# DecaYale/RNNPose

Measured on AMD Instinct MI355X. Metric: pose-refine iters/sec (640x480, B=8, 3x8 recurrent), higher is better.
Workload: dtype f32 (convolutions and volume build: fp16x3-split MFMA, fp32-class accuracy; LM: f64)

## Files before the change

### include/rnnpose_hip.h

```cpp
#ifndef RNNPOSE_HIP_H
#define RNNPOSE_HIP_H

#include <stddef.h>
#include <stdint.h>

#ifdef __cplusplus
extern "C" {
#endif

typedef void* rnnpose_stream_t;

#define RNNPOSE_ABI_VERSION 4
#define RNNPOSE_MAX_LEVELS 4

int rnnpose_abi_version(void);
const char* rnnpose_last_error(void);
int rnnpose_device_info(int dev, char* h_name, int name_len, int* h_cus);

int rnnpose_corr_pyramid_layout(int B, int h, int w, int levels, int64_t* h_offsets ,
                                int* h_hl , int* h_wl );
int rnnpose_corr_pyramid_f32(const float* fmap1, const float* fmap2, int B, int C, int h, int w,
                             int levels, float* pyramid, rnnpose_stream_t stream);
size_t rnnpose_corr_pyramid_f16x3_workspace_bytes(int B, int C, int h, int w);
int rnnpose_corr_pyramid_f16x3(const float* fmap1, const float* fmap2, int layout, int B, int C, int h, int w, int levels,
// ... 191 lines not shown
                             long long ldo, rnnpose_stream_t stream);
long long rnnpose_point_norm_workspace_bytes(int n, int c);
int rnnpose_point_norm_stats_f32(const float* x, int n, int c, long long ldx, float eps, void* workspace, long long workspace_bytes,
                                 float* mean_rstd, rnnpose_stream_t stream);
int rnnpose_point_norm_apply_f32(const float* x, int n, int c, long long ldx, const float* mean_rstd, const float* res, long long ldr,
                                 const float* res_mean_rstd, int leaky, float slope, float* out, long long ldo,
                                 rnnpose_stream_t stream);
int rnnpose_point_maxpool_f32(const float* x, int n_s, int c, long long ldx, const int* idx, int n_q, int width, float* out,
                              long long ldo, rnnpose_stream_t stream);
int rnnpose_point_gather_rows_f32(const float* x, int n_s, int c, long long ldx, const int* idx, int n_q, int idx_ld, float* out,
                                  long long ldo, rnnpose_stream_t stream);
int rnnpose_point_l2_normalize_f32(const float* x, int n, int c, long long ldx, float* out, long long ldo, rnnpose_stream_t stream);
int rnnpose_grid_voxel_keys_f32(const float* points, int n, float ox, float oy, float oz, float dl, long long nx, long long ny,
                                long long* keys, rnnpose_stream_t stream);
int rnnpose_radius_count_f32(const float* queries, int n_q, const float* supports, const int* q_start, const int* s_start,
                             int n_clouds, float radius, int* counts, rnnpose_stream_t stream);
int rnnpose_radius_neighbors_f32(const float* queries, int n_q, const float* supports, const int* q_start, const int* s_start,
                                 int n_clouds, float radius, const long long* offsets, int* cand_idx, float* cand_d2, int width,
                                 int* out, rnnpose_stream_t stream);
size_t rnnpose_conv1x1_resident_packed_bytes(int c_in);
int rnnpose_conv1x1_resident_pack_f16x3(const float* weight, int c_out, int c_in, float w_scale, void* packed,
                                        rnnpose_stream_t stream);
int rnnpose_conv1x1_resident_f16x3(const float* x, int x_c_stride, int x_c_offset, int c_in, const void* w_packed,
                                   const float* bias, float a_scale, float w_scale, int relu, long long n_pixels, float* dst,
                                   int dst_c_stride, int dst_c_offset, int dst_split, rnnpose_stream_t stream);
int rnnpose_corr_lookup_convc1_f16x3(const float* pyramid, const float* coords, int B, int b0, int b1, int h, int w, int levels,
                                     int radius, const void* w_packed, const float* bias, float a_scale, float w_scale, int relu,
                                     float* dst, int dst_c_stride, int dst_c_offset, int dst_split, rnnpose_stream_t stream);
size_t rnnpose_mask_upsample_packed_bytes(void);
int rnnpose_mask_upsample_pack_f16x3(const float* weight, float post_scale, float w_scale, void* packed, rnnpose_stream_t stream);
int rnnpose_mask_upsample_f16x3(const float* x, int x_c_stride, int x_c_offset, const void* w_packed, int c_out,
                                const float* bias, float a_scale, float w_scale, const float* flow_lr, int B, int h, int w,
                                float* flow_up, rnnpose_stream_t stream);

size_t rnnpose_instnorm_workspace_bytes(int B, int HW, int C);
int rnnpose_instnorm_nhwc_f32(const float* x, int B, int HW, int C, float eps, int relu, const float* residual,
                              void* workspace, size_t workspace_bytes, float* mean_rstd, float* out,
                              rnnpose_stream_t stream);
int rnnpose_instnorm_tiles_nhwc_f32(const float* x, int B, int HW, int C, float eps, int relu, const float* residual,
                                    const float* residual_mean_rstd, int residual_relu, const double* tile_stats,
                                    int tiles_per_image, float* mean_rstd, float* out,
                                    rnnpose_stream_t stream);

int rnnpose_nn_search_f32(const float* ref_pts, const float* que_pts, int* idxs, int b, int pn1, int pn2, int dim,
                          int exclude_self, rnnpose_stream_t stream);
void findNearestPointIdxLauncher(float* ref_pts, float* que_pts, int* idxs, int b, int pn1, int pn2, int dim,
                                 int exclude_self);

size_t rnnpose_pose_metrics_workspace_bytes(int B, int P);
int rnnpose_pose_metrics_f64(const float* model, int P, const float* pose_pred, const float* pose_gt, const float* K, int B,
                             int symmetric, void* workspace, size_t workspace_bytes, double* out, rnnpose_stream_t stream);

size_t rnnpose_bop_sym_dist_workspace_bytes(int B, int S);
int rnnpose_bop_sym_dist_f64(const float* model, int P, const float* sym, int S, const float* pose_est, const float* pose_gt,
                             const float* K, int B, void* workspace, size_t workspace_bytes, double* out, rnnpose_stream_t stream);
size_t rnnpose_bop_vsd_workspace_bytes(int B, int H, int W, int NT);
int rnnpose_bop_vsd_f64(const float* depth_est, const float* depth_gt, const float* depth_obs, int S_obs, const int* src_index,
                        const float* K, const float* diameter, int B, int H, int W, double delta, const double* taus, int NT,
                        void* workspace, size_t workspace_bytes, long long* counts, double* err, rnnpose_stream_t stream);

size_t rnnpose_pointcloud_depth_workspace_bytes(int B, int H, int W);
int rnnpose_pointcloud_depth_f32(const float* verts, const int* vert_offsets, int max_verts, const float* T, const float* K, int B,
                                 int H, int W, void* workspace, size_t workspace_bytes, float* out, rnnpose_stream_t stream);
int rnnpose_mask_bbox_f32(const float* depth, int B, int H, int W, int* bbox, rnnpose_stream_t stream);
int rnnpose_zoom_crop_params_f32(const int* bbox, const float* K, const float* T, int B, int H, int W, int crop_h, int crop_w,
                                 float margin_ratio, float* theta, float* K_crop, rnnpose_stream_t stream);
// ... 33 lines not shown
```

### rnnpose_amd/_lib.py

```python
from __future__ import annotations

import ctypes as C
import os

_PKG = os.path.dirname(os.path.abspath(__file__))
ABI_VERSION = 4
LIB_PATH = os.environ.get("RNNPOSE_LIB") or os.path.join(_PKG, "lib", "librnnpose_hip.so")

_p = C.c_void_p
_i = C.c_int
_f = C.c_float
_d = C.c_double
_z = C.c_size_t
_ll = C.c_longlong

class ConvSrc(C.Structure):
    _fields_ = [("ptr", C.c_void_p), ("c_stride", C.c_int), ("c_offset", C.c_int), ("c_count", C.c_int)]


class ConvDesc(C.Structure):
    _fields_ = [("src", ConvSrc * 4), ("n_src", C.c_int), ("B", C.c_int), ("H", C.c_int), ("W", C.c_int),
                ("kh", C.c_int), ("kw", C.c_int), ("stride", C.c_int), ("w_packed", C.c_void_p), ("bias", C.c_void_p),
                ("c_out", C.c_int), ("a_scale", C.c_float), ("w_scale", C.c_float), ("epilogue", C.c_int),
                ("dst", C.c_void_p), ("dst_c_stride", C.c_int), ("dst_c_offset", C.c_int),
# ... 67 lines not shown
    "rnnpose_corr_lookup_nhwc_part_f32": (_i, [_p, _p, _i, _i, _i, _i, _i, _i, _i, _p, _p]),
    "rnnpose_nchw_to_nhwc_f32": (_i, [_p, _i, _i, _i, _p, _i, _i, _p]),
    "rnnpose_nhwc_to_nchw_f32": (_i, [_p, _i, _i, _i, _i, _i, _p, _p]),
    "rnnpose_flow_prep_f32": (_i, [_p, _i, _i, _i, _i, _p, _p, _i, _i, _p]),
    "rnnpose_flow_conv7x7_relu_f32": (_i, [_p, _p, _p, _i, _i, _i, _i, _p, _i, _i, _p]),
    "rnnpose_flow_features_f32": (_i, [_p, _i, _p, _p, _i, _i, _i, _i, _p, _i, _i, _p, _i, _i, _i, _i, _f, _p]),
    "rnnpose_flow_features_induced_f32": (_i, [_p, _p, _p, _i, _i, _f, _p, _p, _i, _i, _i, _i, _p, _i, _i, _p, _i, _i, _i, _i, _f, _p]),
    "rnnpose_corr_lookup_induced_nhwc_part_f32": (_i, [_p, _p, _p, _p, _i, _i, _f, _i, _i, _i, _i, _i, _i, _i, _p, _p, _p]),
    "rnnpose_split_hl_f32": (_i, [_p, _i, _i, _ll, _i, _f, _p, _i, _i, _p]),
    "rnnpose_maxpool2x2_nhwc_f32": (_i, [_p, _i, _i, _i, _i, _i, _i, _p, _i, _i, _p]),
    "rnnpose_upsample2x_bilinear_nhwc_f32": (_i, [_p, _i, _i, _i, _i, _i, _i, _p, _i, _p, _i, _i, _p]),
    "rnnpose_pixel_head_nhwc_f32": (_i, [_p, _i, _i, _i, _i, _i, _p, _i, _p, _p, _i, _i, _p, _p]),
    "rnnpose_point_row_sum_f32": (_i, [_p, _i, _i, _ll, _p, _p]),
    "rnnpose_kpconv_aggregate_f32": (_i, [_p, _i, _p, _i, _p, _i, _p, _i, _f, _p, _i, _ll, _p, _p, _p]),
    "rnnpose_point_linear_f32": (_i, [_p, _i, _i, _ll, _p, _i, _p, _p, _ll, _p]),
    "rnnpose_point_norm_workspace_bytes": (_ll, [_i, _i]),
    "rnnpose_point_norm_stats_f32": (_i, [_p, _i, _i, _ll, _f, _p, _ll, _p, _p]),
    "rnnpose_point_norm_apply_f32": (_i, [_p, _i, _i, _ll, _p, _p, _ll, _p, _i, _f, _p, _ll, _p]),
    "rnnpose_point_maxpool_f32": (_i, [_p, _i, _i, _ll, _p, _i, _i, _p, _ll, _p]),
    "rnnpose_point_gather_rows_f32": (_i, [_p, _i, _i, _ll, _p, _i, _i, _p, _ll, _p]),
    "rnnpose_point_l2_normalize_f32": (_i, [_p, _i, _i, _ll, _p, _ll, _p]),
    "rnnpose_grid_voxel_keys_f32": (_i, [_p, _i, _f, _f, _f, _f, _ll, _ll, _p, _p]),
    "rnnpose_radius_count_f32": (_i, [_p, _i, _p, _p, _p, _i, _f, _p, _p]),
    "rnnpose_radius_neighbors_f32": (_i, [_p, _i, _p, _p, _p, _i, _f, _p, _p, _p, _i, _p, _p]),
    "rnnpose_flow_head_out_f32": (_i, [_p, _i, _i, _i, _p, _p, _p, _i, _i, _i, _p, _p, _p, _p]),
    "rnnpose_convex_upsample_nhwc_f32": (_i, [_p, _p, _i, _i, _i, _p, _p]),
    "rnnpose_mask_upsample_f16x3": (_i, [_p, _i, _i, _p, _i, _p, _f, _f, _p, _i, _i, _i, _p, _p]),
    "rnnpose_mask_upsample_packed_bytes": (_z, []),
    "rnnpose_conv1x1_resident_packed_bytes": (_z, [_i]),
    "rnnpose_conv1x1_resident_pack_f16x3": (_i, [_p, _i, _i, _f, _p, _p]),
    "rnnpose_conv1x1_resident_f16x3": (_i, [_p, _i, _i, _i, _p, _p, _f, _f, _i, _ll, _p, _i, _i, _i, _p]),
    "rnnpose_corr_lookup_convc1_f16x3": (_i, [_p, _p, _i, _i, _i, _i, _i, _i, _i, _p, _p, _f, _f, _i, _p, _i, _i, _i, _p]),
    "rnnpose_mask_upsample_pack_f16x3": (_i, [_p, _f, _f, _p, _p]),
    "rnnpose_instnorm_workspace_bytes": (_z, [_i, _i, _i]),
    "rnnpose_instnorm_tiles_nhwc_f32": (_i, [_p, _i, _i, _i, _f, _i, _p, _p, _i, _p, _i, _p, _p, _p]),
    "rnnpose_instnorm_nhwc_f32": (_i, [_p, _i, _i, _i, _f, _i, _p, _p, _z, _p, _p, _p]),
    "rnnpose_nn_search_f32": (_i, [_p, _p, _p, _i, _i, _i, _i, _i, _p]),
    "findNearestPointIdxLauncher": (None, [_p, _p, _p, _i, _i, _i, _i, _i]),
    "rnnpose_pointcloud_depth_workspace_bytes": (_z, [_i, _i, _i]),
    "rnnpose_pointcloud_depth_f32": (_i, [_p, _p, _i, _p, _p, _i, _i, _i, _p, _z, _p, _p]),
    "rnnpose_mask_bbox_f32": (_i, [_p, _i, _i, _i, _p, _p]),
    "rnnpose_zoom_crop_params_f32": (_i, [_p, _p, _p, _i, _i, _i, _i, _i, _f, _p, _p, _p]),
    "rnnpose_zoom_crop_f32": (_i, [_p, _p, _i, _i, _i, _i, _i, _i, _p, _p, _p]),
    "rnnpose_zoom_crop_indexed_f32": (_i, [_p, _p, _p, _i, _i, _i, _i, _i, _i, _i, _p, _p, _p]),
    "rnnpose_raster_workspace_bytes": (_z, [_i, _i, _i]),
    "rnnpose_raster_mesh_f32": (_i, [_p, _p, _p, _p, _p, _i, _p, _p, _i, _i, _i, _f, _f, _i, _p, _z, _p]),
    "rnnpose_raster_resolve_f32": (_i, [_p, _p, _p, _p, _p, _p, _i, _i, _i, _f, _f, _i, _p, _p, _p, _i, _p, _i, _i, _f, _p, _p, _p, _p]),
    "rnnpose_raster_resolve_tex_f32": (_i, [_p, _p, _p, _p, _p, _p, _i, _i, _i, _f, _f, _i, _p, _p, _p, _i, _p, _p, _p, _p, _p, _p, _p, _p,
                                            _i, _f, _p, _p, _p, _p]),
    "rnnpose_raster_occlusion_f32": (_i, [_p, _p, _p, _p, _p, _i, _p, _p, _i, _i, _i, _f, _f, _p, _p, _i, _f, _p, _p, _z, _p, _p, _p, _p]),
    "rnnpose_pose_metrics_workspace_bytes": (_z, [_i, _i]),
    "rnnpose_pose_metrics_f64": (_i, [_p, _i, _p, _p, _p, _i, _i, _p, _z, _p, _p]),
    "rnnpose_bop_sym_dist_workspace_bytes": (_z, [_i, _i]),
    "rnnpose_bop_sym_dist_f64": (_i, [_p, _i, _p, _i, _p, _p, _p, _i, _p, _z, _p, _p]),
    "rnnpose_bop_vsd_workspace_bytes": (_z, [_i, _i, _i, _i]),
    "rnnpose_bop_vsd_f64": (_i, [_p, _p, _p, _i, _p, _p, _p, _i, _i, _i, _d, _p, _i, _p, _z, _p, _p, _p]),
}

_lib = None


def load() -> C.CDLL:
    global _lib
    if _lib is not None:
        return _lib
    if not os.path.exists(LIB_PATH):
# ... 30 lines not shown
```

### rnnpose_amd/build.py

```python
from __future__ import annotations

import glob
import hashlib
import os
import subprocess
import sys

PKG = os.path.dirname(os.path.abspath(__file__))
ROOT = os.path.dirname(PKG)
CSRC = os.path.join(PKG, "csrc")
LIBDIR = os.path.join(PKG, "lib")
LIB = os.path.join(LIBDIR, "librnnpose_hip.so")
STAMP = os.path.join(LIBDIR, "librnnpose_hip.stamp")
ARCH = "gfx950"
FLAGS = ["-O3", "-std=c++17", "-fPIC", "-shared", f"--offload-arch={ARCH}", "-fno-gpu-rdc", "-Wall",
         "-Wno-unused-function", "-Wno-unused-variable", "-DNDEBUG", "-fno-slp-vectorize"]
PER_FILE_FLAGS = {}
FLAGS += os.environ.get("RNNPOSE_HIPCC_EXTRA", "").split()


def sources():
    return sorted(glob.glob(os.path.join(CSRC, "*.hip")))


TRAFFIC_KERNEL_FILES = ("conv_igemm.hip", "conv_strip.hip", "conv_strip_r32.hip", "conv_strip_r96.hip", "conv_strip_p1.hip", "corr_pyramid.hip")


def source_digest() -> str:
    h = hashlib.sha256()
    files = [os.path.join(CSRC, f) for f in TRAFFIC_KERNEL_FILES] + sorted(glob.glob(os.path.join(CSRC, "*.hpp"))) + \
        sorted(glob.glob(os.path.join(CSRC, "*.cuh")))
    for f in files:
        h.update(os.path.relpath(f, ROOT).encode())
        with open(f, "rb") as fh:
            h.update(fh.read())
    h.update(" ".join(FLAGS).encode())
    h.update(repr(sorted((k, v) for k, v in PER_FILE_FLAGS.items() if k in TRAFFIC_KERNEL_FILES)).encode())
    return h.hexdigest()


def _digest() -> str:
    h = hashlib.sha256()
    files = sources() + sorted(glob.glob(os.path.join(CSRC, "*.hpp"))) + sorted(glob.glob(os.path.join(CSRC, "*.cuh")))
    files.append(os.path.join(ROOT, "include", "rnnpose_hip.h"))
    for f in files:
        h.update(os.path.relpath(f, ROOT).encode())
        with open(f, "rb") as fh:
            h.update(fh.read())
    h.update(" ".join(FLAGS).encode())
    h.update(repr(sorted(PER_FILE_FLAGS.items())).encode())
    return h.hexdigest()


def hipcc() -> str:
    for c in (os.environ.get("HIPCC"), "/opt/rocm/bin/hipcc", "hipcc"):
        if c and (os.path.isabs(c) and os.path.exists(c) or not os.path.isabs(c)):
            return c
    raise RuntimeError("hipcc not found")


def build(force: bool = False, verbose: bool = False) -> str:
    import fcntl
    os.makedirs(LIBDIR, exist_ok=True)
    dig = _digest()
    if not force and os.path.exists(LIB) and os.path.exists(STAMP) and open(STAMP).read().strip() == dig:
        return LIB
    with open(os.path.join(LIBDIR, ".build.lock"), "w") as lock:
        fcntl.flock(lock, fcntl.LOCK_EX)
        try:
            if not force and os.path.exists(LIB) and os.path.exists(STAMP) and open(STAMP).read().strip() == dig:
                return LIB
            return _build_locked(dig, verbose)
        finally:
            fcntl.flock(lock, fcntl.LOCK_UN)


# ... 41 lines not shown
```

### rnnpose_amd/csrc/nhwc_ops.hip

```cpp
#define RP_CONTRACT_LOCAL 1
#include "common.hpp"
#include "f16x3.cuh"
#include "induced.cuh"

namespace {

__global__ __launch_bounds__(256) void nchw_to_nhwc_kernel(const float* __restrict__ src, float* __restrict__ dst, int C,
                                                           int HW, int dst_cs, int dst_co) {
  __shared__ float tile[32][33];
  const int b = blockIdx.z;
  const int p0 = blockIdx.x * 32, c0 = blockIdx.y * 32;
  const int tx = threadIdx.x & 31, ty = threadIdx.x >> 5;
#pragma unroll
  for (int r = 0; r < 4; ++r) {
    const int c = c0 + ty + 8 * r, pp = p0 + tx;
    tile[ty + 8 * r][tx] = (c < C && pp < HW) ? src[(static_cast<long long>(b) * C + c) * HW + pp] : 0.f;
  }
  __syncthreads();
#pragma unroll
  for (int r = 0; r < 4; ++r) {
    const int pp = p0 + ty + 8 * r, c = c0 + tx;
    if (c < C && pp < HW) dst[(static_cast<long long>(b) * HW + pp) * dst_cs + dst_co + c] = tile[tx][ty + 8 * r];
  }
}
// ... 1342 lines not shown

int rnnpose_grid_voxel_keys_f32(const float* points, int n, float ox, float oy, float oz, float dl, long long nx, long long ny,
                                long long* keys, rnnpose_stream_t stream) {
  const char* fn = "rnnpose_grid_voxel_keys_f32";
  RP_REQUIRE(points && keys, fn, "null pointer");
  RP_REQUIRE(n > 0 && dl > 0.f && nx > 0 && ny > 0, fn, "bad size (n, nx, ny > 0, dl > 0)");
  hipLaunchKernelGGL(grid_keys_kernel, dim3(rp::cdiv(n, 256)), dim3(256), 0, rp::as_stream(stream), points, n, ox, oy, oz, dl, nx, ny,
                     reinterpret_cast<i64*>(keys));
  return rp::check_launch(fn);
}

int rnnpose_radius_count_f32(const float* queries, int n_q, const float* supports, const int* q_start, const int* s_start,
                             int n_clouds, float radius, int* counts, rnnpose_stream_t stream) {
  const char* fn = "rnnpose_radius_count_f32";
  RP_REQUIRE(queries && supports && q_start && s_start && counts, fn, "null pointer");
  RP_REQUIRE(n_q > 0 && n_clouds > 0, fn, "bad size (n_q, n_clouds > 0)");
  hipLaunchKernelGGL(radius_kernel<0>, dim3(rp::cdiv(n_q, 256)), dim3(256), 0, rp::as_stream(stream), queries, n_q, supports, q_start,
                     s_start, n_clouds, radius, counts, nullptr, nullptr, nullptr, 0, nullptr);
  return rp::check_launch(fn);
}

int rnnpose_radius_neighbors_f32(const float* queries, int n_q, const float* supports, const int* q_start, const int* s_start,
                                 int n_clouds, float radius, const long long* offsets, int* cand_idx, float* cand_d2, int width,
                                 int* out, rnnpose_stream_t stream) {
  const char* fn = "rnnpose_radius_neighbors_f32";
  RP_REQUIRE(queries && supports && q_start && s_start && offsets && cand_idx && cand_d2 && out, fn, "null pointer");
  RP_REQUIRE(n_q > 0 && n_clouds > 0 && width > 0, fn, "bad size (n_q, n_clouds, width > 0)");
  hipLaunchKernelGGL(radius_kernel<1>, dim3(rp::cdiv(n_q, 256)), dim3(256), 0, rp::as_stream(stream), queries, n_q, supports, q_start,
                     s_start, n_clouds, radius, nullptr, reinterpret_cast<const i64*>(offsets), cand_idx, cand_d2, width, out);
  return rp::check_launch(fn);
}

}
```

### rnnpose_amd/engine.py

```python
from __future__ import annotations

import torch

from . import env, ops, streams


class UpdateEngine:
    def __init__(self, update_block):
        self.blk = update_block
        self._key = None
        self._w = None
        self._buf_key = None
        self._b = None
        self._sets = {}
        self.epoch = 0
        self._ksws = {}
        self.split_batch = env.flag("RNNPOSE_SPLIT_BATCH", True)
        self.side_stream = env.flag("RNNPOSE_SIDE_STREAM", False)
        self.parts = env.number("RNNPOSE_PARTS", 2)
        self.parts_forced = env.text("RNNPOSE_PARTS") is not None
        self.fused_mask = env.flag("RNNPOSE_FUSED_MASK", True)
        self.resident_1x1 = env.flag("RNNPOSE_RESIDENT_1X1", True)
        self.fused_lookup = env.flag("RNNPOSE_FUSED_LOOKUP", False)
        self.fused_induced = env.flag("RNNPOSE_FUSED_INDUCED", False)
        self.ksplit = env.flag("RNNPOSE_KSPLIT", True)
        self.hl = env.flag("RNNPOSE_SPLIT_TENSORS", True)
        self.single_product = False
        self.tile = {k: int(v) for k, v in (kv.split("=") for kv in filter(None, env.text("RNNPOSE_CONV_TILE", "").split(",")))}

    def _params(self):
        b = self.blk
        e, g = b.encoder, b.gru
        return [e.convc1, e.convc2, e.convf1, e.convf2, e.conv, g.convz1, g.convr1, g.convq1, g.convz2, g.convr2,
                g.convq2, b.flow_head.conv1, b.flow_head.conv2, b.mask[0], b.mask[2]]

    def param_key(self):
        return ops.param_key(self._params())

    def refresh(self):
        self._weights()
        return self._key

    def _weights(self):
        key = self.param_key()
        if key == self._key:
            return self._w
        b = self.blk
        e, g = b.encoder, b.gru
        cat = lambda *t: torch.cat([x.detach() for x in t], 0)
        hm = lambda wt: torch.cat([wt[:, :128], wt[:, 256:]], 1).contiguous()
        zero = lambda n: torch.zeros(n, device=g.convz1.weight.device, dtype=torch.float32)
        P = ops.PackedConv
        w = dict(
            convc1=P(e.convc1.weight, e.convc1.bias, [e.convc1.weight.shape[1]]),
            convc1r=ops.PackedConv1x1(e.convc1.weight, e.convc1.bias) if ops.PackedConv1x1.fits(e.convc1.weight) else None,
            convc2=P(e.convc2.weight, e.convc2.bias, [256]),
            convf1_wt=e.convf1.weight.detach().float().reshape(e.convf1.weight.shape[0], 98).t().contiguous(),
            convf1_b=e.convf1.bias.detach().float().contiguous(),
            convf2=P(e.convf2.weight, e.convf2.bias, [128]),
            conv=P(e.conv.weight, e.conv.bias, [256]),
            zr=P(hm(cat(g.convz1.weight, g.convr1.weight)), cat(g.convz1.bias, g.convr1.bias), [128, 128]),
            q=P(hm(g.convq1.weight), g.convq1.bias, [128, 128]),
            zr2=P(hm(cat(g.convz2.weight, g.convr2.weight)), cat(g.convz2.bias, g.convr2.bias), [128, 128]),
            q2=P(hm(g.convq2.weight), g.convq2.bias, [128, 128]),
            inp1=P(cat(g.convz1.weight, g.convr1.weight, g.convq1.weight)[:, 128:256].contiguous(), zero(384), [128]),
            inp2=P(cat(g.convz2.weight, g.convr2.weight, g.convq2.weight)[:, 128:256].contiguous(), zero(384), [128]),
            heads=P(cat(b.flow_head.conv1.weight, b.mask[0].weight), cat(b.flow_head.conv1.bias, b.mask[0].bias), [128]),
            mask2=P(b.mask[2].weight, b.mask[2].bias, [256], post_scale=0.25),
            mask2u=ops.PackedMaskHead(b.mask[2].weight, b.mask[2].bias, post_scale=0.25),
            flow2_w=b.flow_head.conv2.weight.detach().float().contiguous(),
            flow2_b=b.flow_head.conv2.bias.detach().float().contiguous(),
        )
        self._key, self._w = key, w
        return w

    MAX_SETS = 4

    def _buffers(self, B, h, w, device):
        key = (B, h, w, str(device))
        if key != self._buf_key:
            st = self._sets.pop(key, None)
            if st is None:
                z = lambda c: torch.zeros(B, h, w, c, device=device, dtype=torch.float32)
                st = dict(corr=z(324), cor1=z(256), corflo=z(256), flow4=z(4), flo1=z(128), motion=z(128), hA=z(128),
                          hB=z(128), inp=z(128), inp1=z(384), inp2=z(384), z=z(128), rh=z(128), heads=z(512), delta=z(2), flow_lr=z(2),
                          mask=z(576), coords1=torch.zeros(B, 2, h, w, device=device))
                if self.hl:
                    st.update(hA_s=z(128), hB_s=z(128), inp_s=z(128))
                if len(self._sets) >= self.MAX_SETS:
                    self._sets.pop(next(iter(self._sets)))
                    self.epoch += 1
            self._sets[key] = st
# ... 85 lines not shown

    def step(self, corr_fn, coords1, tail=None, flow_up=None):
        B, _, h, w = coords1.shape
        main = torch.cuda.current_stream()
        if flow_up is None:
            flow_up = torch.empty(B, 2, 8 * h, 8 * w, device=coords1.device, dtype=torch.float32)
        hv = self.halves(B)

        def half(b0, b1, st):
            yield from self.half_gen(corr_fn, coords1[b0:b1], B, b0, b1, st, flow_up[b0:b1], single=len(hv) == 1)
            if tail is not None:
                tail(b0, b1, flow_up[b0:b1])

        jobs = []
        for i, (b0, b1) in enumerate(hv):
            st = main if i == 0 else streams.helper_stream(coords1.device, i)
            jobs.append((half(b0, b1, st), st))
        streams.run_interleaved(jobs, main)
        return self._b["coords1"], flow_up

    def _chain_gen(self, W, b, coords1, main, side, flow_is_delta=False, want_mask=False, have_cor1=False, induced=None):
        mask_here = want_mask or not self.fused_mask
        hl = self.hl
        tl = self.tile.get
        R = ops.EPI_RELU

        ks_main = b.get("_ksws")
        ks_side = b.get("_ksws_side") if side is not None else ks_main

        def c(name, srcs, dst, epi, hl_out=False, ks=None, **kw):
            ops.conv2d_nhwc(W[name], srcs, dst, epi, src_hl=hl, dst_hl=hl and hl_out, tile=tl(name, 0),
                            ksplit_ws=ks_main if ks is None else ks, single_product=self.single_product, **kw)
        def flow_chain():
            if induced is not None:
                ops.flow_features_induced(induced, W["convf1_wt"], W["convf1_b"], b["flo1"], b["motion"], 126, out_split=hl, motion_split=hl,
                                          a_scale=ops.A_SCALE)
            else:
                ops.flow_features(coords1, W["convf1_wt"], W["convf1_b"], b["flo1"], b["motion"], 126, subtract_grid=not flow_is_delta,
                                  out_split=hl, motion_split=hl, a_scale=ops.A_SCALE)
            yield
            c("convf2", [(b["flo1"], 0)], (b["corflo"], 192), R, hl_out=True, ks=ks_side)
            yield

        join = None
        if side is None:
            yield from flow_chain()
        else:
            join = streams.side_branch(main, side, lambda: streams.drain(flow_chain()))
        if have_cor1:
            pass
        elif self.resident_1x1 and W["convc1r"] is not None:
            ops.conv1x1_resident(W["convc1r"], (b["corr"], 0), (b["cor1"], 0), relu=True, dst_split=hl)
            yield
        else:
            ops.conv2d_nhwc(W["convc1"], [(b["corr"], 0)], (b["cor1"], 0), R, dst_hl=hl, single_product=self.single_product)
            yield
        c("convc2", [(b["cor1"], 0)], (b["corflo"], 0), R, hl_out=True)
        yield
        if join is not None:
            main.wait_event(join)
        c("conv", [(b["corflo"], 0)], (b["motion"], 0), R, hl_out=True)
        yield
        hs = (lambda k: b[k + "_s"]) if hl else (lambda k: b[k])
        hx = lambda hbuf: [(hbuf, 0), (b["motion"], 0)]
        sp = (lambda k: dict(dst_split=(b[k + "_s"], 0))) if hl else (lambda k: {})
        c("zr", hx(hs("hA")), (b["z"], 0), ops.EPI_GRU_ZR, aux0=(b["hA"], 0), dst2=(b["rh"], 0), dst2_hl=hl, gru_c=128, add_map=(b["inp1"], 0))
# ... 165 lines not shown
```

### rnnpose_amd/ops.py

```python
from __future__ import annotations

import ctypes as C
from contextlib import contextmanager

import torch

from . import _lib, env

F32 = torch.float32
F64 = torch.float64

_prof = None


_event_pool = []


@contextmanager
def profile(names=None):
    global _prof
    prev = _prof
    rec = {"_only": set(names) if names else None, "_next": 0}
    _prof = rec
    try:
# ... 814 lines not shown
    _launch("rnnpose_nchw_to_nhwc_f32", _ptr(src), B, Cc, H * W, _ptr(dst), dst.shape[3], c_offset, _stream())
    return dst


def nhwc_to_nchw(src, c_offset: int = 0, c_count: int | None = None, out=None):
    B, H, W, Cs = src.shape
    c_count = Cs - c_offset if c_count is None else c_count
    dst = out if out is not None else torch.empty(B, c_count, H, W, device=src.device, dtype=F32)
    _launch("rnnpose_nhwc_to_nchw_f32", _ptr(src), B, c_count, H * W, Cs, c_offset, _ptr(dst), _stream())
    return dst


def flow_prep(coords1, flow4, motion, motion_c_offset, subtract_grid: bool = True):
    B, _, h, w = coords1.shape
    _launch("rnnpose_flow_prep_f32", _ptr(coords1), int(subtract_grid), B, h, w, _ptr(flow4), _ptr(motion), motion.shape[3],
            motion_c_offset, _stream())


def flow_conv7x7_relu(flow4, w_t, bias, out, out_c_offset=0):
    B, h, w, _ = flow4.shape
    c_out = w_t.shape[1]
    _launch("rnnpose_flow_conv7x7_relu_f32", _ptr(flow4), _ptr(w_t), _ptr(bias), B, h, w, c_out, _ptr(out), out.shape[-1],
            out_c_offset, _stream(), work=2.0 * 98 * c_out * B * h * w)
    return out


def flow_features(coords1, w_t, bias, out, motion, motion_c_offset, out_c_offset=0, subtract_grid: bool = True,
                  out_split: bool = False, motion_split: bool = False, a_scale: float = 8.0):
    B, _, h, w = coords1.shape
    c_out = w_t.shape[1]
    _launch("rnnpose_flow_features_f32", _ptr(coords1), int(subtract_grid), _ptr(w_t), _ptr(bias), B, h, w, c_out, _ptr(out),
            out.shape[-1], out_c_offset, _ptr(motion), motion.shape[3], motion_c_offset, int(bool(out_split)), int(bool(motion_split)),
            float(a_scale), _stream(), work=2.0 * 98 * c_out * B * h * w)
    return out


def split_hl(src, dst=None, src_c_offset: int = 0, c_count: int | None = None, dst_c_offset: int = 0, a_scale: float = 8.0):
    _nhwc(src, "src")
    B, H, W, Cs = src.shape
    c_count = Cs - src_c_offset if c_count is None else c_count
    if dst is None:
        dst = torch.empty(B, H, W, c_count, device=src.device, dtype=F32)
    _lib.call("rnnpose_split_hl_f32", _ptr(src), Cs, int(src_c_offset), B * H * W, int(c_count), float(a_scale), _ptr(dst),
              dst.shape[3], int(dst_c_offset), _stream())
    return dst


def unsplit_hl(t, a_scale: float = 8.0):
    sh = t.shape
    v = t.contiguous().view(torch.float16).view(*sh[:-1], sh[-1] // 8, 2, 8).float()
    return ((v[..., 0, :] + v[..., 1, :]) / a_scale).reshape(sh)


def flow_head_out(x, x_c_offset, c_in, weight, bias, coords1, delta, coords1_out, flow_lr):
    B, h, w, cs = x.shape
    _launch("rnnpose_flow_head_out_f32", _ptr(x), cs, x_c_offset, c_in, _ptr(weight), _ptr(bias), _ptr(coords1), B, h, w,
            _ptr(delta), _ptr(coords1_out), _ptr(flow_lr), _stream())


def convex_upsample_nhwc(flow_lr, mask, out=None):
    B, h, w, _ = mask.shape
    if out is None:
        out = torch.empty(B, 2, 8 * h, 8 * w, device=mask.device, dtype=F32)
    _launch("rnnpose_convex_upsample_nhwc_f32", _ptr(flow_lr), _ptr(mask), B, h, w, _ptr(out), _stream(),
            nbytes=4.0 * B * h * w * (576 + 2 + 128))
    return out
# ... 753 lines not shown
```

Before: 770.7.

## Fuse convf1 7x7 and convf2 3x3 flow branch into one MFMA kernel

Adds a kernel that computes the 7x7 flow-feature conv and the following 3x3 conv in one pass per spatial tile. The 128-channel intermediate stays in LDS with a halo, using fp16x3-split MFMA for both stages, and the motion channels are written directly. This removes the round trip of the flo1 intermediate through global memory and one kernel launch. In exchange the halo region is recomputed for each tile, and the kernel uses a lot of LDS and registers, which limits occupancy. It is enabled by default through RNNPOSE_FUSED_FLOW_BRANCH.

```diff
diff --git a/include/rnnpose_hip.h b/include/rnnpose_hip.h
--- a/include/rnnpose_hip.h
+++ b/include/rnnpose_hip.h
@@ -247,6 +247,14 @@
 int rnnpose_mask_upsample_f16x3(const float* x, int x_c_stride, int x_c_offset, const void* w_packed, int c_out,
                                 const float* bias, float a_scale, float w_scale, const float* flow_lr, int B, int h, int w,
                                 float* flow_up, rnnpose_stream_t stream);
+size_t rnnpose_flow_branch_packed_bytes(void);
+int rnnpose_flow_branch_patch_rows(int rows);
+int rnnpose_flow_branch_pack_f16x3(const float* w1_oihw, float w1_scale, const float* w2_oihw, float w2_scale, void* packed,
+                                   rnnpose_stream_t stream);
+int rnnpose_flow_branch_f16x3(const float* coords1, int subtract_grid, const void* w_packed, int c_mid, int c_out, const float* bias1,
+                              const float* bias2, float a_scale, float w1_scale, float w2_scale, int B, int h, int w, float* out,
+                              int out_c_stride, int out_c_offset, int out_split, float* motion, int motion_c_stride, int motion_c_offset,
+                              int motion_split, rnnpose_stream_t stream);
 
 size_t rnnpose_instnorm_workspace_bytes(int B, int HW, int C);
 int rnnpose_instnorm_nhwc_f32(const float* x, int B, int HW, int C, float eps, int relu, const float* residual,
diff --git a/rnnpose_amd/_lib.py b/rnnpose_amd/_lib.py
--- a/rnnpose_amd/_lib.py
+++ b/rnnpose_amd/_lib.py
@@ -123,6 +123,10 @@
     "rnnpose_conv1x1_resident_f16x3": (_i, [_p, _i, _i, _i, _p, _p, _f, _f, _i, _ll, _p, _i, _i, _i, _p]),
     "rnnpose_corr_lookup_convc1_f16x3": (_i, [_p, _p, _i, _i, _i, _i, _i, _i, _i, _p, _p, _f, _f, _i, _p, _i, _i, _i, _p]),
     "rnnpose_mask_upsample_pack_f16x3": (_i, [_p, _f, _f, _p, _p]),
+    "rnnpose_flow_branch_packed_bytes": (_z, []),
+    "rnnpose_flow_branch_patch_rows": (_i, [_i]),
+    "rnnpose_flow_branch_pack_f16x3": (_i, [_p, _f, _p, _f, _p, _p]),
+    "rnnpose_flow_branch_f16x3": (_i, [_p, _i, _p, _i, _i, _p, _p, _f, _f, _f, _i, _i, _i, _p, _i, _i, _i, _p, _i, _i, _i, _p]),
     "rnnpose_instnorm_workspace_bytes": (_z, [_i, _i, _i]),
     "rnnpose_instnorm_tiles_nhwc_f32": (_i, [_p, _i, _i, _i, _f, _i, _p, _p, _i, _p, _i, _p, _p, _p]),
     "rnnpose_instnorm_nhwc_f32": (_i, [_p, _i, _i, _i, _f, _i, _p, _p, _z, _p, _p, _p]),
diff --git a/rnnpose_amd/build.py b/rnnpose_amd/build.py
--- a/rnnpose_amd/build.py
+++ b/rnnpose_amd/build.py
@@ -19,8 +19,15 @@
 FLAGS += os.environ.get("RNNPOSE_HIPCC_EXTRA", "").split()
 
 
+INCLUDED_SOURCES = {"flow_branch.hip": "nhwc_ops.hip"}
+
+
+def all_sources():
+    return sorted(glob.glob(os.path.join(CSRC, "*.hip")))
+
+
 def sources():
-    return sorted(glob.glob(os.path.join(CSRC, "*.hip")))
+    return [f for f in all_sources() if os.path.basename(f) not in INCLUDED_SOURCES]
 
 
 TRAFFIC_KERNEL_FILES = ("conv_igemm.hip", "conv_strip.hip", "conv_strip_r32.hip", "conv_strip_r96.hip", "conv_strip_p1.hip", "corr_pyramid.hip")
@@ -41,7 +48,7 @@
 
 def _digest() -> str:
     h = hashlib.sha256()
-    files = sources() + sorted(glob.glob(os.path.join(CSRC, "*.hpp"))) + sorted(glob.glob(os.path.join(CSRC, "*.cuh")))
+    files = all_sources() + sorted(glob.glob(os.path.join(CSRC, "*.hpp"))) + sorted(glob.glob(os.path.join(CSRC, "*.cuh")))
     files.append(os.path.join(ROOT, "include", "rnnpose_hip.h"))
     for f in files:
         h.update(os.path.relpath(f, ROOT).encode())
diff --git a/rnnpose_amd/csrc/flow_branch.hip b/rnnpose_amd/csrc/flow_branch.hip
--- /dev/null
+++ b/rnnpose_amd/csrc/flow_branch.hip
@@ -0,0 +1,391 @@
+#include <algorithm>
+
+#include "common.hpp"
+#include "f16x3.cuh"
+
+#ifndef FB_ABL
+#define FB_ABL 0
+#endif
+
+namespace {
+namespace flowbr {
+
+using rp::f32x16;
+using rp::h4;
+using rp::h8;
+
+constexpr int TW = 16;
+constexpr int FW = 24;
+constexpr int HWD = TW + 2;
+constexpr int PS = 136;
+constexpr int CM = 128, CO = 64;
+constexpr int K1STEPS = 7, K2STEPS = 72;
+constexpr int W1_HALFS = K1STEPS * 4 * 64 * 8;
+constexpr int W2_HALFS = K2STEPS * 2 * 64 * 8;
+
+template <int TH>
+struct Geo {
+  static constexpr int FH = TH + 8;
+  static constexpr int HH = TH + 2;
+  static constexpr int NHALO = HH * HWD;
+  static constexpr int MT1 = (NHALO + 31) / 32;
+  static constexpr int MT2 = TH * TW / 32;
+  static constexpr int P = TH * TW;
+  static constexpr int HPLANE = MT1 * 32 * PS;
+  static constexpr int FPLANE = 2 * FH * FW;
+  static constexpr int LDS = (2 * HPLANE + 4 * FPLANE) * 2;
+  static constexpr int RING = TH == 8 ? 4 : 8;
+  static_assert(P * CO * sizeof(float) <= 2 * HPLANE * sizeof(_Float16), "the partial tile reuses the flo1 planes");
+};
+
+__host__ __device__ constexpr int f1_rowoff(int r, int FH) { return ((r / 7) * FH + (r % 7)) * FW; }
+
+template <int TH>
+__global__ __launch_bounds__(256, TH == 4 ? 2 : 1) void flow_branch_kernel(const float* __restrict__ coords1, int subtract_grid, const uint4* __restrict__ wp,
+                                                          const float* __restrict__ bias1, const float* __restrict__ bias2, float a_scale,
+                                                          float os1, float os2, int h, int w, int tiles_x, int tiles_y,
+                                                          float* __restrict__ out, int ocs, int oco, int out_hl, float* __restrict__ motion,
+                                                          int mcs, int mco, int motion_hl, unsigned long long* __restrict__ sat) {
+#pragma clang fp contract(off)
+  using G = Geo<TH>;
+  __shared__ __attribute__((aligned(16))) unsigned char smem[G::LDS];
+  _Float16* const sH = reinterpret_cast<_Float16*>(smem);
+  _Float16* const sF = sH + 2 * G::HPLANE;
+  const unsigned tid = threadIdx.x, lane = tid & 63u, wave = __builtin_amdgcn_readfirstlane(tid >> 6);
+  const unsigned l31 = lane & 31u, lh = lane >> 5;
+
+  unsigned t = blockIdx.x;
+  const unsigned tx_ = t % static_cast<unsigned>(tiles_x);
+  t /= static_cast<unsigned>(tiles_x);
+  const unsigned ty_ = t % static_cast<unsigned>(tiles_y), b = t / static_cast<unsigned>(tiles_y);
+  const int y0 = static_cast<int>(ty_) * TH, x0 = static_cast<int>(tx_) * TW;
+  const unsigned n = static_cast<unsigned>(h) * static_cast<unsigned>(w);
+  bool sflag = false;
+
+  {
+    constexpr int NE = (G::FH * FW + 255) / 256;
+    float vx[NE], vy[NE];
+    bool ok[NE];
+#pragma unroll
+    for (int j = 0; j < NE; ++j) {
+      const unsigned e_ = tid + 256u * j, e = e_ < static_cast<unsigned>(G::FH * FW) ? e_ : static_cast<unsigned>(G::FH * FW - 1);
+      const int iy = y0 - 4 + static_cast<int>(e / FW), ix = x0 - 4 + static_cast<int>(e % FW);
+      ok[j] = static_cast<unsigned>(iy) < static_cast<unsigned>(h) && static_cast<unsigned>(ix) < static_cast<unsigned>(w);
+      const unsigned off = ok[j] ? static_cast<unsigned>(iy) * static_cast<unsigned>(w) + static_cast<unsigned>(ix) : 0u;
+      vx[j] = coords1[b * 2u * n + off];
+      vy[j] = coords1[(b * 2u + 1u) * n + off];
+    }
+    __builtin_amdgcn_sched_barrier(0);
+#pragma unroll
+    for (int j = 0; j < NE; ++j) {
+      const unsigned e = tid + 256u * j;
+      if (e >= static_cast<unsigned>(G::FH * FW)) break;
+      const unsigned fy = e / FW, fx = e % FW;
+      const int iy = y0 - 4 + static_cast<int>(fy), ix = x0 - 4 + static_cast<int>(fx);
+      float2 v = make_float2(0.f, 0.f);
+      if (ok[j]) {
+        v.x = vx[j] - (subtract_grid ? static_cast<float>(ix) : 0.f);
+        v.y = vy[j] - (subtract_grid ? static_cast<float>(iy) : 0.f);
+      }
+      h4 hi, lo;
+      const float4 q = make_float4(v.x, v.y, 0.f, 0.f);
+      rp::split4(q, a_scale, hi, lo);
+      sF[e] = hi.x;
+      sF[G::FH * FW + e] = hi.y;
+      sF[G::FPLANE + e] = lo.x;
+      sF[G::FPLANE + G::FH * FW + e] = lo.y;
+      if (fx) {
+        sF[2 * G::FPLANE + e - 1u] = hi.x;
+        sF[2 * G::FPLANE + G::FH * FW + e - 1u] = hi.y;
+        sF[3 * G::FPLANE + e - 1u] = lo.x;
+        sF[3 * G::FPLANE + G::FH * FW + e - 1u] = lo.y;
+      }
+      if (ok[j] && fy >= 4u && fy < 4u + TH && fx >= 4u && fx < 4u + TW) {
+        sflag |= rp::quad_saturates(q, a_scale);
+        float* mrow = motion + (b * n + static_cast<unsigned>(iy) * static_cast<unsigned>(w) + static_cast<unsigned>(ix)) * static_cast<unsigned>(mcs);
+        if (motion_hl) {
+          _Float16* ph = reinterpret_cast<_Float16*>(mrow + (mco & ~7)) + (mco & 7);
+          *reinterpret_cast<rp::h2*>(ph) = rp::h2{hi.x, hi.y};
+          *reinterpret_cast<rp::h2*>(ph + 8) = rp::h2{lo.x, lo.y};
+        } else {
+          *reinterpret_cast<float2*>(mrow + mco) = v;
+        }
+      }
+    }
+  }
+
+  const unsigned kh = wave >> 1, nt = wave & 1u;
+  const uint4* const w2h = wp + (2 * W1_HALFS) / 8;
+  const uint4* const w2l = w2h + W2_HALFS / 8;
+  constexpr int RING = G::RING, NI = K2STEPS / 2;
+  uint4 Bh[RING], Bl[RING];
+  auto load_b = [&](int i) {
+    const unsigned o = ((2u * i + kh) * 2u + nt) * 64u + lane;
+    Bh[i % RING] = w2h[o];
+    Bl[i % RING] = w2l[o];
+  };
+#pragma unroll
+  for (int i = 0; i < RING - 1; ++i) load_b(i);
+
+  {
+    uint4 b1h[K1STEPS], b1l[K1STEPS];
+#pragma unroll
+    for (int kk = 0; kk < K1STEPS; ++kk) {
+      b1h[kk] = wp[(kk * 4 + wave) * 64u + lane];
+      b1l[kk] = wp[W1_HALFS / 8 + (kk * 4 + wave) * 64u + lane];
+    }
+    const float bss = bias1[32u * wave + l31] * a_scale, os1s = os1 * a_scale;
+    unsigned inw[G::MT1];
+#pragma unroll
+    for (int mt = 0; mt < G::MT1; ++mt) {
+      const unsigned m = 32u * mt + l31, qy = m / HWD, qx = m - qy * HWD;
+      const int iy = y0 - 1 + static_cast<int>(qy), ix = x0 - 1 + static_cast<int>(qx);
+      const bool in = m < static_cast<unsigned>(G::NHALO) && static_cast<unsigned>(iy) < static_cast<unsigned>(h) && static_cast<unsigned>(ix) < static_cast<unsigned>(w);
+      unsigned bits = in ? 1u << l31 : 0u;
+#pragma unroll
+      for (int o = 1; o < 32; o <<= 1) bits |= static_cast<unsigned>(__shfl_xor(static_cast<int>(bits), o));
+      inw[mt] = bits;
+    }
+    __syncthreads();
+    const unsigned* const f32 = reinterpret_cast<const unsigned*>(sF);
+    uint4 Ah[2][K1STEPS], Al[2][K1STEPS];
+    f32x16 acc1[2];
+    auto load_a = [&](int mt, uint4 (&ahq)[K1STEPS], uint4 (&alq)[K1STEPS]) {
+      const unsigned m_ = 32u * mt + l31, m = m_ < static_cast<unsigned>(G::NHALO) ? m_ : static_cast<unsigned>(G::NHALO - 1);
+      const unsigned hy = m / HWD, hx = m - hy * HWD;
+      const unsigned pb = hy * FW + (hx & ~1u) + ((hx & 1u) ? 2u * G::FPLANE : 0u);
+#pragma unroll
+      for (int kk = 0; kk < K1STEPS; ++kk) {
+        const unsigned d = (pb + (lh ? f1_rowoff(2 * kk + 1, G::FH) : f1_rowoff(2 * kk, G::FH))) >> 1;
+        ahq[kk] = make_uint4(f32[d], f32[d + 1], f32[d + 2], f32[d + 3] & 0xffffu);
+        alq[kk] = make_uint4(f32[G::FPLANE / 2 + d], f32[G::FPLANE / 2 + d + 1], f32[G::FPLANE / 2 + d + 2], f32[G::FPLANE / 2 + d + 3] & 0xffffu);
+      }
+    };
+    auto mfmas = [&](const uint4 (&ahq)[K1STEPS], const uint4 (&alq)[K1STEPS], f32x16& acc) {
+#pragma unroll
+      for (int r = 0; r < 16; ++r) acc[r] = 0.f;
+#pragma unroll
+      for (int kk = 0; kk < ((FB_ABL & 1) ? 0 : K1STEPS); ++kk) {
+        const h8 ah = __builtin_bit_cast(h8, ahq[kk]), al = __builtin_bit_cast(h8, alq[kk]);
+        const h8 Bhh = __builtin_bit_cast(h8, b1h[kk]), Bll = __builtin_bit_cast(h8, b1l[kk]);
+        acc = __builtin_amdgcn_mfma_f32_32x32x16_f16(al, Bhh, acc, 0, 0, 0);
+        acc = __builtin_amdgcn_mfma_f32_32x32x16_f16(ah, Bll, acc, 0, 0, 0);
+        acc = __builtin_amdgcn_mfma_f32_32x32x16_f16(ah, Bhh, acc, 0, 0, 0);
+      }
+    };
+    auto epilogue = [&](int mt, const f32x16& acc) {
+      const unsigned wv = inw[mt] >> (4u * lh);
+      _Float16* const rowp = sH + (32u * mt + 4u * lh) * PS + 32u * wave + l31;
+#pragma unroll
+      for (int g = 0; g < ((FB_ABL & 2) ? 0 : 4); ++g) {
+        float y[4];
+#pragma unroll
+        for (int e = 0; e < 4; ++e) {
+          const float v = fmaxf(__builtin_fmaf(acc[4 * g + e], os1s, bss), 0.f);
+          y[e] = ((wv >> (e + 8 * g)) & 1u) ? v : 0.f;
+        }
+        h4 hi, lo;
+        const float4 q = make_float4(y[0], y[1], y[2], y[3]);
+        rp::split4(q, 1.0f, hi, lo);
+        sflag |= rp::quad_saturates(q, 1.0f);
+#pragma unroll
+        for (int e = 0; e < 4; ++e) {
+          rowp[(e + 8 * g) * PS] = hi[e];
+          rowp[G::HPLANE + (e + 8 * g) * PS] = lo[e];
+        }
+      }
+    };
+    load_a(0, Ah[0], Al[0]);
+#pragma unroll
+    for (int mt = 0; mt < G::MT1; ++mt) {
+      if (mt + 1 < G::MT1) load_a(mt + 1, Ah[(mt + 1) & 1], Al[(mt + 1) & 1]);
+      mfmas(Ah[mt & 1], Al[mt & 1], acc1[mt & 1]);
+      if (mt > 0) epilogue(mt - 1, acc1[(mt - 1) & 1]);
+    }
+    epilogue(G::MT1 - 1, acc1[(G::MT1 - 1) & 1]);
+  }
+  __syncthreads();
+
+  f32x16 acc[G::MT2];
+#pragma unroll
+  for (int mt = 0; mt < G::MT2; ++mt)
+#pragma unroll
+    for (int r = 0; r < 16; ++r) acc[mt][r] = 0.f;
+  {
+    const unsigned pb = ((l31 >> 4) * HWD + (l31 & 15u)) * PS + 8u * lh + 16u * kh;
+    h8 ah[2][G::MT2], al[2][G::MT2];
+    auto load_a2 = [&](int i, h8 (&hq)[G::MT2], h8 (&lq)[G::MT2]) {
+      const int tap = i >> 2, ty = tap / 3, tx = tap % 3;
+      const unsigned ao = pb + static_cast<unsigned>((ty * HWD + tx) * PS + 32 * (i & 3));
+#pragma unroll
+      for (int mt = 0; mt < G::MT2; ++mt) {
+        hq[mt] = *reinterpret_cast<const h8*>(sH + ao + mt * (2 * HWD * PS));
+        lq[mt] = *reinterpret_cast<const h8*>(sH + G::HPLANE + ao + mt * (2 * HWD * PS));
+      }
+    };
+    if (!(FB_ABL & 4)) load_a2(0, ah[0], al[0]);
+#pragma unroll
+    for (int i = 0; i < ((FB_ABL & 4) ? 0 : NI); ++i) {
+      if (i + RING - 1 < NI && !(FB_ABL & 16)) load_b(i + RING - 1);
+      if (i + 1 < NI) load_a2(i + 1, ah[(i + 1) & 1], al[(i + 1) & 1]);
+      const h8 Bhh = __builtin_bit_cast(h8, Bh[i % RING]), Bll = __builtin_bit_cast(h8, Bl[i % RING]);
+#pragma unroll
+      for (int mt = 0; mt < G::MT2; ++mt) acc[mt] = __builtin_amdgcn_mfma_f32_32x32x16_f16(al[i & 1][mt], Bhh, acc[mt], 0, 0, 0);
+#pragma unroll
+      for (int mt = 0; mt < G::MT2; ++mt) acc[mt] = __builtin_amdgcn_mfma_f32_32x32x16_f16(ah[i & 1][mt], Bll, acc[mt], 0, 0, 0);
+#pragma unroll
+      for (int mt = 0; mt < G::MT2; ++mt) acc[mt] = __builtin_amdgcn_mfma_f32_32x32x16_f16(ah[i & 1][mt], Bhh, acc[mt], 0, 0, 0);
+    }
+  }
+  __syncthreads();
+
+  float* const R = reinterpret_cast<float*>(smem);
+  {
+    if (kh == 1u && !(FB_ABL & 8)) {
+#pragma unroll
+      for (int mt = 0; mt < G::MT2; ++mt)
+#pragma unroll
+        for (int r = 0; r < 16; ++r) R[(32u * mt + (r & 3) + 8u * (r >> 2) + 4u * lh) * CO + 32u * nt + l31] = acc[mt][r];
+    }
+    __syncthreads();
+    if (kh == 0u && !(FB_ABL & 8)) {
+#pragma unroll
+      for (int mt = 0; mt < G::MT2; ++mt)
+#pragma unroll
+        for (int r = 0; r < 16; ++r) {
+          float* const q = R + (32u * mt + (r & 3) + 8u * (r >> 2) + 4u * lh) * CO + 32u * nt + l31;
+          *q = acc[mt][r] + *q;
+        }
+    }
+    __syncthreads();
+  }
+  {
+    const unsigned g = tid & 7u;
+    const float4 ba = *reinterpret_cast<const float4*>(bias2 + 8u * g), bb = *reinterpret_cast<const float4*>(bias2 + 8u * g + 4u);
+#pragma unroll
+    for (int j = 0; j < G::P * 8 / 256; ++j) {
+      const unsigned p = (tid >> 3) + 32u * j;
+      const int iy = y0 + static_cast<int>(p >> 4), ix = x0 + static_cast<int>(p & 15u);
+      const float4 a0 = *reinterpret_cast<const float4*>(R + p * CO + 8u * g), a1 = *reinterpret_cast<const float4*>(R + p * CO + 8u * g + 4u);
+      const float4 y0q = make_float4(fmaxf(__builtin_fmaf(a0.x, os2, ba.x), 0.f), fmaxf(__builtin_fmaf(a0.y, os2, ba.y), 0.f),
+                                     fmaxf(__builtin_fmaf(a0.z, os2, ba.z), 0.f), fmaxf(__builtin_fmaf(a0.w, os2, ba.w), 0.f));
+      const float4 y1q = make_float4(fmaxf(__builtin_fmaf(a1.x, os2, bb.x), 0.f), fmaxf(__builtin_fmaf(a1.y, os2, bb.y), 0.f),
+                                     fmaxf(__builtin_fmaf(a1.z, os2, bb.z), 0.f), fmaxf(__builtin_fmaf(a1.w, os2, bb.w), 0.f));
+      if (iy >= h || ix >= w) continue;
+      float* o = out + (b * n + static_cast<unsigned>(iy) * static_cast<unsigned>(w) + static_cast<unsigned>(ix)) * static_cast<unsigned>(ocs) + static_cast<unsigned>(oco) + 8u * g;
+      if (out_hl) {
+        h4 h0, l0, h1, l1;
+        rp::split4(y0q, a_scale, h0, l0);
+        rp::split4(y1q, a_scale, h1, l1);
+        sflag |= rp::quad_saturates(y0q, a_scale) || rp::quad_saturates(y1q, a_scale);
+        *reinterpret_cast<h8*>(o) = h8{h0.x, h0.y, h0.z, h0.w, h1.x, h1.y, h1.z, h1.w};
+        *reinterpret_cast<h8*>(o + 4) = h8{l0.x, l0.y, l0.z, l0.w, l1.x, l1.y, l1.z, l1.w};
+      } else {
+        *reinterpret_cast<float4*>(o) = y0q;
+        *reinterpret_cast<float4*>(o + 4) = y1q;
+      }
+    }
+  }
+  if (sat && sflag) atomicAdd(sat, 1ull);
+}
+
+__global__ void flow_branch_pack_kernel(const float* __restrict__ w1, float s1, const float* __restrict__ w2, float s2, _Float16* __restrict__ packed) {
+  const int i = blockIdx.x * blockDim.x + threadIdx.x;
+  if (i >= W1_HALFS + W2_HALFS) return;
+  float v;
+  _Float16 *hi, *lo;
+  if (i < W1_HALFS) {
+    const int j = i & 7, ln = (i >> 3) & 63, nt = (i >> 9) & 3, kk = i >> 11;
+    const int r = 2 * kk + (ln >> 5), co = 32 * nt + (ln & 31);
+    v = j < 7 ? w1[((co * 2 + r / 7) * 7 + r % 7) * 7 + j] * s1 : 0.f;
+    hi = packed + i;
+    lo = packed + W1_HALFS + i;
+  } else {
+    const int k = i - W1_HALFS;
+    const int j = k & 7, ln = (k >> 3) & 63, nt = (k >> 9) & 1, ks = k >> 10;
+    const int tap = ks >> 3, ci = 16 * (ks & 7) + 8 * (ln >> 5) + j, co = 32 * nt + (ln & 31);
+    v = w2[(co * CM + ci) * 9 + tap] * s2;
+    hi = packed + 2 * W1_HALFS + k;
+    lo = packed + 2 * W1_HALFS + W2_HALFS + k;
+  }
+  const _Float16 hv = static_cast<_Float16>(v);
+  *hi = hv;
+  *lo = static_cast<_Float16>(v - static_cast<float>(hv));
+}
+
+template <int TH>
+int launch(const char* fn, const float* coords1, int subtract_grid, const void* wp, const float* bias1, const float* bias2, float a_scale, float w1_scale,
+           float w2_scale, int B, int h, int w, float* out, int ocs, int oco, int out_hl, float* motion, int mcs, int mco, int motion_hl,
+           hipStream_t st) {
+  const int tiles_x = rp::cdiv(w, TW), tiles_y = rp::cdiv(h, TH);
+  const long long blocks = static_cast<long long>(B) * tiles_x * tiles_y;
+  hipLaunchKernelGGL(flow_branch_kernel<TH>, dim3(static_cast<unsigned>(blocks)), dim3(256), 0, st, coords1, subtract_grid,
+                     static_cast<const uint4*>(wp), bias1, bias2, a_scale, 1.0f / (a_scale * w1_scale), 1.0f / (a_scale * w2_scale), h, w,
+                     tiles_x, tiles_y, out, ocs, oco, out_hl, motion, mcs, mco, motion_hl, rp::sat_counter());
+  return rp::check_launch(fn);
+}
+
+}
+}
+
+static int g_flow_branch_rows = 0;
+
+extern "C" {
+
+int rnnpose_flow_branch_patch_rows(int rows) {
+  if (rows != 0 && rows != 4 && rows != 8) return rp::fail_arg("rnnpose_flow_branch_patch_rows", "rows must be 0, 4 or 8");
+  g_flow_branch_rows = rows;
+  return 0;
+}
+
+size_t rnnpose_flow_branch_packed_bytes(void) { return static_cast<size_t>(2 * (flowbr::W1_HALFS + flowbr::W2_HALFS)) * sizeof(_Float16); }
+
+int rnnpose_flow_branch_pack_f16x3(const float* w1_oihw, float w1_scale, const float* w2_oihw, float w2_scale, void* packed,
+                                   rnnpose_stream_t stream) {
+  const char* fn = "rnnpose_flow_branch_pack_f16x3";
+  RP_REQUIRE(w1_oihw && w2_oihw && packed && w1_scale > 0.f && w2_scale > 0.f, fn, "null pointer / non-positive scale");
+  RP_REQUIRE(reinterpret_cast<uintptr_t>(packed) % 16 == 0, fn, "packed weights must be 16-byte aligned");
+  const int total = flowbr::W1_HALFS + flowbr::W2_HALFS;
+  hipLaunchKernelGGL(flowbr::flow_branch_pack_kernel, dim3(rp::cdiv(total, 256)), dim3(256), 0, rp::as_stream(stream), w1_oihw, w1_scale, w2_oihw,
+                     w2_scale, static_cast<_Float16*>(packed));
+  return rp::check_launch(fn);
+}
+
+int rnnpose_flow_branch_f16x3(const float* coords1, int subtract_grid, const void* w_packed, int c_mid, int c_out, const float* bias1,
+                              const float* bias2, float a_scale, float w1_scale, float w2_scale, int B, int h, int w, float* out,
+                              int out_c_stride, int out_c_offset, int out_split, float* motion, int motion_c_stride, int motion_c_offset,
+                              int motion_split, rnnpose_stream_t stream) {
+  const char* fn = "rnnpose_flow_branch_f16x3";
+  RP_REQUIRE(coords1 && w_packed && bias1 && bias2 && out && motion, fn, "null pointer");
+  RP_REQUIRE(c_mid == flowbr::CM && c_out == flowbr::CO, fn, "the kernel takes convf1 with 128 and convf2 with 64 output channels");
+  RP_REQUIRE(B > 0 && h > 0 && w > 0 && a_scale > 0.f && w1_scale > 0.f && w2_scale > 0.f, fn, "bad size / scale");
+  RP_REQUIRE(reinterpret_cast<uintptr_t>(w_packed) % 16 == 0 && reinterpret_cast<uintptr_t>(bias2) % 16 == 0 &&
+                 reinterpret_cast<uintptr_t>(coords1) % 4 == 0 && reinterpret_cast<uintptr_t>(bias1) % 4 == 0,
+             fn, "packed weights / bias2 must be 16-byte aligned");
+  RP_REQUIRE(out_c_offset >= 0 && out_c_offset + flowbr::CO <= out_c_stride && motion_c_offset >= 0 && motion_c_offset % 2 == 0 &&
+                 motion_c_stride % 2 == 0 && motion_c_offset + 2 <= motion_c_stride,
+             fn, "bad output windows");
+  if (out_split)
+    RP_REQUIRE(out_c_offset % 8 == 0 && out_c_stride % 8 == 0 && reinterpret_cast<uintptr_t>(out) % 32 == 0, fn,
+               "split-form out: channel offset / stride multiples of 8, 32-byte aligned");
+  else
+    RP_REQUIRE(out_c_offset % 4 == 0 && out_c_stride % 4 == 0 && reinterpret_cast<uintptr_t>(out) % 16 == 0, fn,
+               "fp32 out: channel offset / stride multiples of 4, 16-byte aligned");
+  if (motion_split)
+    RP_REQUIRE(motion_c_stride % 8 == 0 && reinterpret_cast<uintptr_t>(motion) % 32 == 0, fn,
+               "split-form motion: channel stride multiple of 8, 32-byte aligned");
+  else
+    RP_REQUIRE(reinterpret_cast<uintptr_t>(motion) % 8 == 0, fn, "fp32 motion: 8-byte aligned");
+  const long long px = static_cast<long long>(B) * h * w;
+  RP_REQUIRE(h < 32768 && w < 32768 && px * std::max(out_c_stride, motion_c_stride) < (1LL << 31) && 2 * px < (1LL << 31), fn,
+             "tensor too large for 32-bit indices");
+  hipStream_t st = rp::as_stream(stream);
+  const int rows = g_flow_branch_rows ? g_flow_branch_rows : 4;
+  if (rows == 4)
+    return flowbr::launch<4>(fn, coords1, subtract_grid, w_packed, bias1, bias2, a_scale, w1_scale, w2_scale, B, h, w, out, out_c_stride, out_c_offset,
+                     out_split, motion, motion_c_stride, motion_c_offset, motion_split, st);
+  return flowbr::launch<8>(fn, coords1, subtract_grid, w_packed, bias1, bias2, a_scale, w1_scale, w2_scale, B, h, w, out, out_c_stride, out_c_offset,
+                   out_split, motion, motion_c_stride, motion_c_offset, motion_split, st);
+}
+
+}
diff --git a/rnnpose_amd/csrc/nhwc_ops.hip b/rnnpose_amd/csrc/nhwc_ops.hip
--- a/rnnpose_amd/csrc/nhwc_ops.hip
+++ b/rnnpose_amd/csrc/nhwc_ops.hip
@@ -1398,3 +1398,5 @@
 }
 
 }
+
+#include "flow_branch.hip"
diff --git a/rnnpose_amd/engine.py b/rnnpose_amd/engine.py
--- a/rnnpose_amd/engine.py
+++ b/rnnpose_amd/engine.py
@@ -23,6 +23,7 @@
         self.resident_1x1 = env.flag("RNNPOSE_RESIDENT_1X1", True)
         self.fused_lookup = env.flag("RNNPOSE_FUSED_LOOKUP", False)
         self.fused_induced = env.flag("RNNPOSE_FUSED_INDUCED", False)
+        self.fused_flow_branch = env.flag("RNNPOSE_FUSED_FLOW_BRANCH", True)
         self.ksplit = env.flag("RNNPOSE_KSPLIT", True)
         self.hl = env.flag("RNNPOSE_SPLIT_TENSORS", True)
         self.single_product = False
@@ -58,6 +59,8 @@
             convf1_wt=e.convf1.weight.detach().float().reshape(e.convf1.weight.shape[0], 98).t().contiguous(),
             convf1_b=e.convf1.bias.detach().float().contiguous(),
             convf2=P(e.convf2.weight, e.convf2.bias, [128]),
+            flowbr=(ops.PackedFlowBranch(e.convf1.weight, e.convf1.bias, e.convf2.weight, e.convf2.bias)
+                    if ops.PackedFlowBranch.fits(e.convf1.weight, e.convf2.weight) else None),
             conv=P(e.conv.weight, e.conv.bias, [256]),
             zr=P(hm(cat(g.convz1.weight, g.convr1.weight)), cat(g.convz1.bias, g.convr1.bias), [128, 128]),
             q=P(hm(g.convq1.weight), g.convq1.bias, [128, 128]),
@@ -209,6 +212,11 @@
             ops.conv2d_nhwc(W[name], srcs, dst, epi, src_hl=hl, dst_hl=hl and hl_out, tile=tl(name, 0),
                             ksplit_ws=ks_main if ks is None else ks, single_product=self.single_product, **kw)
         def flow_chain():
+            if self.fused_flow_branch and not self.single_product and W["flowbr"] is not None:
+                ops.flow_branch(W["flowbr"], coords1, b["corflo"], b["motion"], 126, out_c_offset=192, subtract_grid=not flow_is_delta,
+                                out_split=hl, motion_split=hl)
+                yield
+                return
             if induced is not None:
                 ops.flow_features_induced(induced, W["convf1_wt"], W["convf1_b"], b["flo1"], b["motion"], 126, out_split=hl, motion_split=hl,
                                           a_scale=ops.A_SCALE)
diff --git a/rnnpose_amd/ops.py b/rnnpose_amd/ops.py
--- a/rnnpose_amd/ops.py
+++ b/rnnpose_amd/ops.py
@@ -870,6 +870,47 @@
     _launch("rnnpose_flow_features_f32", _ptr(coords1), int(subtract_grid), _ptr(w_t), _ptr(bias), B, h, w, c_out, _ptr(out),
             out.shape[-1], out_c_offset, _ptr(motion), motion.shape[3], motion_c_offset, int(bool(out_split)), int(bool(motion_split)),
             float(a_scale), _stream(), work=2.0 * 98 * c_out * B * h * w)
+    return out
+
+
+class PackedFlowBranch:
+
+    @staticmethod
+    def fits(w1, w2) -> bool:
+        return tuple(w1.shape) == (128, 2, 7, 7) and tuple(w2.shape) == (64, 128, 3, 3)
+
+    def __init__(self, w1, b1, w2, b2, a_scale: float = 8.0):
+        import math
+        range_guard_arm(w1.device)
+        w1, w2 = _chk(w1.detach(), "w1"), _chk(w2.detach(), "w2")
+        if not self.fits(w1, w2):
+            raise ValueError("needs convf1 (128,2,7,7) and convf2 (64,128,3,3)")
+        scale = lambda t: float(2.0 ** math.floor(math.log2(1024.0 / float(t.abs().max())))) if float(t.abs().max()) > 0 else 1.0
+        self.c_mid, self.c_out = int(w1.shape[0]), int(w2.shape[0])
+        self.w1_scale, self.w2_scale, self.a_scale = scale(w1), scale(w2), float(a_scale)
+        self.bias1, self.bias2 = _chk(b1.detach(), "b1").contiguous(), _chk(b2.detach(), "b2").contiguous()
+        n = int(_lib.load().rnnpose_flow_branch_packed_bytes())
+        self.w_packed = torch.empty(n // 2, device=w1.device, dtype=torch.float16)
+        _lib.call("rnnpose_flow_branch_pack_f16x3", _ptr(w1), self.w1_scale, _ptr(w2), self.w2_scale, _ptr(self.w_packed), _stream())
+
+
+_flow_branch_env_applied = False
+
+
+def flow_branch(pf: PackedFlowBranch, coords1, out, motion, motion_c_offset, out_c_offset=0, subtract_grid: bool = True,
+                out_split: bool = False, motion_split: bool = False):
+    global _flow_branch_env_applied
+    if not _flow_branch_env_applied:
+        _flow_branch_env_applied = True
+        rows = env.number("RNNPOSE_FLOW_BRANCH_ROWS", None)
+        if rows is not None:
+            _lib.call("rnnpose_flow_branch_patch_rows", rows)
+    B, _, h, w = coords1.shape
+    n = B * h * w
+    _launch("rnnpose_flow_branch_f16x3", _ptr(coords1), int(subtract_grid), _ptr(pf.w_packed), pf.c_mid, pf.c_out, _ptr(pf.bias1), _ptr(pf.bias2),
+            pf.a_scale, pf.w1_scale, pf.w2_scale, B, h, w, _ptr(out), out.shape[-1], int(out_c_offset), int(bool(out_split)), _ptr(motion),
+            motion.shape[3], int(motion_c_offset), int(bool(motion_split)), _stream(),
+            work=2.0 * n * (98 * 128 + 1152 * 64), nbytes=4.0 * (2 * n + 98 * 128 + 1152 * 64 + 64 * n + 2 * n))
     return out
 
 
```

After: 774.8, median of 6. No clear change (+0.5%).
